# OmerKerner/noLZSS

Hardware: AMD Instinct MI355X
Metric: bases/sec factorized (1 GB sigma=4 DNA) + HBM GB/s fraction (higher is better)
Workload: dtype u32; 1 GPU; dna1g: one 2^30-base synthetic DNA sequence per GPU (sigma=4, 40% copied blocks, 1% substitutions), full factorization to (start,length,ref) records in HBM; bases_per_gpu=1073741824, parallelism=1 independent sequence shard(s), all-gather of counts

## Files before the change

nolzss_amd/csrc/chain.hip:

```cpp
#include "pipeline.hpp"
#include "pyramid.hpp"
#include "scan.hpp"

#include <cassert>

namespace nolzss {
namespace {

constexpr int kThreads = 256;
constexpr int kTile = 4096;
constexpr int kPerThread = kTile / kThreads;
constexpr uint32_t kNone = 0xffffffffu;

constexpr uint32_t kLenMask = 0x7fffffffu;

__device__ __forceinline__ uint32_t next_pos(uint32_t p, uint32_t code, uint32_t n) {
    const uint32_t L = code & kLenMask;
    const uint64_t nx = (uint64_t)p + (L ? L : 1u);
    return nx > n ? n : (uint32_t)nx;
}

__global__ __launch_bounds__(kThreads) void chain_exit_kernel(const uint32_t *__restrict__ lstar, uint32_t n,
                                                              uint32_t start_pos,
                                                              uint32_t *__restrict__ exit0,
                                                              uint32_t *__restrict__ target_bits) {
    __shared__ uint32_t jump[kTile];
    const uint32_t base = blockIdx.x * (uint32_t)kTile;
    const uint32_t tile_end = (n - base < (uint32_t)kTile) ? n : base + kTile;
    const int tid = threadIdx.x;
    uint32_t ls[kPerThread];
#pragma unroll
    for (int j = 0; j < kPerThread; ++j) {
        const uint32_t p = base + j * kThreads + tid;
        ls[j] = lstar[p < n ? p : n - 1u];
    }
#pragma unroll
    for (int j = 0; j < kPerThread; ++j) {
        const uint32_t lp = j * kThreads + tid;
        const uint32_t p = base + lp;
        jump[lp] = (p < n) ? next_pos(p, ls[j], n) : n;
    }
    __syncthreads();
    for (int round = 0; round < 13; ++round) {
        int changed = 0;
#pragma unroll
        for (int j = 0; j < kPerThread; ++j) {
            const uint32_t lp = j * kThreads + tid;
            const uint32_t t = jump[lp];
            if (t < tile_end) {
                jump[lp] = jump[t - base];
                changed = 1;
            }
        }
        if (!__syncthreads_or(changed)) break;
    }
#pragma unroll
    for (int j = 0; j < kPerThread; ++j) {
        const uint32_t lp = j * kThreads + tid;
        const uint32_t p = base + lp;
        if (p < n) {
            const uint32_t e = jump[lp];
            exit0[p] = e;
            const bool last = (lp + 1 == (uint32_t)kTile) || (p + 1 >= n);
            if (e < n && (last || jump[lp + 1] != e)) atomicOr(&target_bits[e >> 5], 1u << (e & 31));
        }
    }
    if (blockIdx.x == 0 && tid == 0 && start_pos < n) atomicOr(&target_bits[start_pos >> 5], 1u << (start_pos & 31));
}

__global__ __launch_bounds__(kThreads) void popcount_kernel(const uint32_t *__restrict__ bits, uint32_t nwords,
                                                            uint32_t *__restrict__ counts) {
    const size_t stride = (size_t)gridDim.x * blockDim.x;
    for (size_t w = (size_t)blockIdx.x * blockDim.x + threadIdx.x; w < nwords; w += stride)
        counts[w] = (uint32_t)__popc(bits[w]);
}

__global__ __launch_bounds__(kThreads) void node_fill_kernel(const uint32_t *__restrict__ bits,
                                                             const uint32_t *__restrict__ prefix, uint32_t nwords,
                                                             uint32_t *__restrict__ node_pos) {
    const size_t stride = (size_t)gridDim.x * blockDim.x;
    for (size_t w = (size_t)blockIdx.x * blockDim.x + threadIdx.x; w < nwords; w += stride) {
        uint32_t b = bits[w];
        uint32_t id = prefix[w];
        while (b) {
            const int bit = __ffs((int)b) - 1;
            node_pos[id++] = (uint32_t)(w * 32 + bit);
            b &= b - 1;
        }
    }
}

__device__ __forceinline__ uint32_t node_id(const uint32_t *bits, const uint32_t *prefix, uint32_t p) {
    return prefix[p >> 5] + (uint32_t)__popc(bits[p >> 5] & ((1u << (p & 31)) - 1u));
}

__global__ __launch_bounds__(kThreads) void node_edges_kernel(const uint32_t *__restrict__ node_pos, uint32_t K,
                                                              const uint32_t *__restrict__ exit0, uint32_t n,
                                                              const uint32_t *__restrict__ bits,
                                                              const uint32_t *__restrict__ prefix,
                                                              uint32_t start_pos, uint32_t *__restrict__ nxt,
                                                              uint32_t *__restrict__ reach) {
    const size_t stride = (size_t)gridDim.x * blockDim.x;
    for (size_t k = (size_t)blockIdx.x * blockDim.x + threadIdx.x; k <= K; k += stride) {
        if (k == K) {
            nxt[k] = K;
            reach[k] = 0;
            continue;
        }
        const uint32_t p = node_pos[k];
        const uint32_t e = exit0[p];
        nxt[k] = (e >= n) ? K : node_id(bits, prefix, e);
        reach[k] = (p == start_pos) ? 1u : 0u;
    }
}

__global__ __launch_bounds__(kThreads) void wyllie_kernel(const uint32_t *__restrict__ nxt_in,
                                                          uint32_t *__restrict__ nxt_out, uint32_t K,
                                                          uint32_t *reach) {
    const size_t stride = (size_t)gridDim.x * blockDim.x;
    for (size_t k = (size_t)blockIdx.x * blockDim.x + threadIdx.x; k < K; k += stride) {
        const uint32_t w = nxt_in[k];
        if (w < K) {
            if (reach[k]) reach[w] = 1u;
            nxt_out[k] = nxt_in[w];
        } else {
            nxt_out[k] = K;
        }
    }
}

__global__ __launch_bounds__(kThreads) void tile_entries_kernel(const uint32_t *__restrict__ node_pos,
                                                                const uint32_t *__restrict__ reach, uint32_t K,
                                                                uint32_t *__restrict__ entry) {
    const size_t stride = (size_t)gridDim.x * blockDim.x;
    for (size_t k = (size_t)blockIdx.x * blockDim.x + threadIdx.x; k < K; k += stride)
        if (reach[k]) {
            const uint32_t p = node_pos[k];
            entry[p / kTile] = p;
        }
}

__global__ __launch_bounds__(64) void chain_mark_kernel(const uint32_t *__restrict__ lstar, uint32_t n,
                                                        const uint32_t *__restrict__ entry,
                                                        unsigned long long *__restrict__ chain_bits,
                                                        uint32_t *__restrict__ tile_count) {
    __shared__ uint16_t jmp[kTile];
    __shared__ unsigned long long bits[kTile / 64];
    const uint32_t base = blockIdx.x * (uint32_t)kTile;
    const uint32_t tile_end = (n - base < (uint32_t)kTile) ? n : base + kTile;
    const int lane = threadIdx.x;
    const uint32_t e = entry[blockIdx.x];
    const size_t word0 = (size_t)blockIdx.x * (kTile / 64);
    if (e == kNone) {
        chain_bits[word0 + lane] = 0ull;
        if (lane == 0) tile_count[blockIdx.x] = 0;
        return;
    }
    constexpr int kBatch = 16;
    for (int j0 = 0; j0 < kTile / 64; j0 += kBatch) {
        uint32_t ls[kBatch];
#pragma unroll
        for (int j = 0; j < kBatch; ++j) {
            const uint32_t p = base + (uint32_t)(j0 + j) * 64u + lane;
            ls[j] = lstar[p < n ? p : n - 1u];
        }
#pragma unroll
        for (int j = 0; j < kBatch; ++j) {
            const uint32_t lp = (uint32_t)(j0 + j) * 64u + lane;
            const uint32_t p = base + lp;
            uint32_t nl = kTile;
            if (p < n) {
                const uint32_t nx = next_pos(p, ls[j], n);
                if (nx < tile_end) nl = nx - base;
            }
            jmp[lp] = (uint16_t)nl;
        }
    }
    bits[lane] = 0ull;
    __syncthreads();
    if (lane == 0) {
        uint32_t p = e - base, cnt = 0;
        while (p < (uint32_t)kTile) {
            bits[p >> 6] |= 1ull << (p & 63);
            ++cnt;
            p = jmp[p];
        }
        tile_count[blockIdx.x] = cnt;
    }
    __syncthreads();
    chain_bits[word0 + lane] = bits[lane];
}

__global__ __launch_bounds__(64) void emit_positions_kernel(const unsigned long long *__restrict__ chain_bits,
                                                            const uint32_t *__restrict__ tile_off,
                                                            uint32_t *__restrict__ fpos) {
    const int lane = threadIdx.x;
    const size_t word = (size_t)blockIdx.x * (kTile / 64) + lane;
    unsigned long long b = chain_bits[word];
    const uint32_t c = (uint32_t)__popcll(b);
    uint32_t off = wave_scan_inclusive(c, OpAdd<uint32_t>()) - c + tile_off[blockIdx.x];
    const uint32_t p0 = blockIdx.x * (uint32_t)kTile + lane * 64u;
    while (b) {
        const int bit = __ffsll((long long)b) - 1;
        fpos[off++] = p0 + (uint32_t)bit;
        b &= b - 1;
    }
}

template <bool kRC>
__global__ __launch_bounds__(kThreads) void length_hist_kernel(const unsigned long long *__restrict__ chain_bits,
                                                               uint32_t nwords, const uint32_t *__restrict__ lstar,
                                                               uint32_t *__restrict__ hist,
                                                               uint64_t *__restrict__ tail,
                                                               uint32_t *__restrict__ tail_count, uint32_t tail_cap) {
    constexpr uint32_t T = kLengthHistBins;
    constexpr uint32_t kBins = kRC ? 2 * T : T;
    __shared__ uint32_t h[kBins];
    for (uint32_t b = threadIdx.x; b < kBins; b += kThreads) h[b] = 0;
    __syncthreads();
    const uint32_t stride = gridDim.x * kThreads;
    for (uint32_t w = blockIdx.x * kThreads + threadIdx.x; w < nwords; w += stride) {
        unsigned long long b = chain_bits[w];
        while (b) {
            const int bit = __ffsll((long long)b) - 1;
            b &= b - 1;
            const uint32_t code = lstar[(size_t)w * 64 + (uint32_t)bit];
            const uint32_t strand = kRC ? (code >> 31) : 0u;
            uint32_t L = code & kLenMask;
            L = L ? L : 1u;
            if (L < T) {
                atomicAdd(&h[strand * T + L], 1u);
            } else {
                const uint32_t slot = atomicAdd(tail_count, 1u);
                assert(slot < tail_cap);
                if (slot < tail_cap) tail[slot] = (uint64_t)L | ((uint64_t)strand << 32);
            }
        }
    }
    __syncthreads();
    for (uint32_t b = threadIdx.x; b < kBins; b += kThreads)
        if (h[b]) atomicAdd(&hist[b], h[b]);
}

__global__ __launch_bounds__(kThreads) void gather_lengths_kernel(uint32_t *__restrict__ fpos, uint32_t z,
                                                                  const uint32_t *__restrict__ lstar) {
    const size_t stride = (size_t)gridDim.x * blockDim.x;
    for (size_t k = (size_t)blockIdx.x * blockDim.x + threadIdx.x; k < z; k += stride) {
        const uint32_t L = lstar[fpos[k]] & kLenMask;
        fpos[k] = L ? L : 1u;
    }
}

constexpr uint32_t kEmitScan = 4;

struct FactorRec {
    uint64_t start, length, ref;
};

template <bool kRC, bool kRebase>
__global__ __launch_bounds__(kThreads) void factor_kernel(const uint32_t *__restrict__ fpos, uint32_t z,
                                                          const uint32_t *__restrict__ lstar,
                                                          const uint32_t *__restrict__ isa,
                                                          const uint32_t *__restrict__ sa,
                                                          const uint32_t *__restrict__ lcp, Pyramid Psa,
                                                          Pyramid Plcp, Pyramid Pmax, uint32_t rcN,
                                                          FactorRec *__restrict__ out, TermTable terms, uint32_t n) {
    const size_t stride = (size_t)gridDim.x * blockDim.x;
    for (size_t k = (size_t)blockIdx.x * blockDim.x + threadIdx.x; k < z; k += stride) {
        const uint32_t i = fpos[k];
        const uint32_t nxt = k + 1 < z ? fpos[k + 1] : n;
        uint32_t code = nxt - i;
        if (kRC || code == 1u) code = lstar[i];
        const uint32_t L = code & kLenMask;
        const bool is_rc = kRC && (code >> 31);
        FactorRec f;
        f.start = i;
        if (L == 0) {
            f.length = 1;
            f.ref = i;
        } else {
            const uint32_t r = isa[i] - 1u;
            uint32_t lo = r, hi = r + 1, steps = 0;
            while (lcp[lo] >= L) {
                --lo;
                if (++steps == kEmitScan) {
                    lo = (uint32_t)pyr_nearest_left<false>(Plcp, lo, L);
                    break;
                }
            }
            steps = 0;
            while (lcp[hi] >= L) {
                ++hi;
                if (++steps == kEmitScan) {
                    hi = pyr_nearest_right<false>(Plcp, hi, L);
                    break;
                }
            }
            hi -= 1;
            f.length = L;
            if (!is_rc) {
                uint32_t mn;
                if (hi - lo < 2 * kEmitScan) {
                    mn = kNone;
                    for (uint32_t q = lo; q <= hi; ++q) {
                        const uint32_t v = sa[q];
                        mn = v < mn ? v : mn;
                    }
                } else {
                    mn = pyr_range<false>(Psa, lo, hi);
                }
                f.ref = mn;
            } else {
                uint32_t mx;
                if (hi - lo < 2 * kEmitScan) {
                    mx = 0;
                    for (uint32_t q = lo; q <= hi; ++q) {
                        const uint32_t v = sa[q];
                        mx = v > mx ? v : mx;
                    }
                } else {
                    mx = pyr_range<true>(Pmax, lo, hi);
                }
                const uint64_t end = 2ull * rcN - mx;
                f.ref = (1ull << 63) | (end - L + 1);
            }
        }
        if (kRebase) {
            const uint32_t t = term_lower_bound(terms, i);
            const uint64_t base = t ? (uint64_t)terms.pos[t - 1] + 1 : 0;
            f.start -= base;
            f.ref -= base;
        }
        out[k] = f;
    }
}

inline unsigned grid_for(size_t items, unsigned cap = 256u * 16u) {
    size_t g = div_up(items, (size_t)kThreads);
    if (g < 1) g = 1;
    return (unsigned)(g > cap ? cap : g);
}

}

uint32_t resolve_chain(Context &ctx, uint32_t n, uint32_t start_pos, const uint32_t *lstar, const uint32_t *sa,
                       const uint32_t *isa, const uint32_t *lcp, const Pyramid &Psa, const Pyramid &Plcp,
                       void **d_factors_out, uint32_t rcN, const Pyramid *Pmax, uint32_t **d_fpos_out,
                       const TermTable *rebase, const ChainLengthsOut *lengths) {
    hipStream_t s = ctx.stream;
    Arena &arena = ctx.arena;
    if (d_factors_out) *d_factors_out = nullptr;
    if (d_fpos_out) *d_fpos_out = nullptr;
    if (start_pos >= n) return 0;

    const uint32_t num_tiles = (uint32_t)div_up(n, kTile);
    const uint32_t tbits_words = (uint32_t)div_up((size_t)n + 1, 32);

    uint32_t *fpos = nullptr;
    const size_t mark = arena.mark();
    uint32_t *exit0 = arena.alloc<uint32_t>(n);
    uint32_t *tbits = arena.alloc<uint32_t>(tbits_words);
    uint32_t *tprefix = arena.alloc<uint32_t>(tbits_words);
    uint32_t *d_total = arena.alloc<uint32_t>(2);
    HIP_CHECK(hipMemsetAsync(tbits, 0, sizeof(uint32_t) * tbits_words, s));
    {
        ProfScope ps(ctx.profiler(), "chain_exit", s);
        chain_exit_kernel<<<num_tiles, kThreads, 0, s>>>(lstar, n, start_pos, exit0, tbits);
        KERNEL_CHECK();
    }
    {
        ProfScope ps(ctx.profiler(), "chain_nodes", s);
        popcount_kernel<<<grid_for(tbits_words), kThreads, 0, s>>>(tbits, tbits_words, tprefix);
        KERNEL_CHECK();
        scan_exclusive_add_u32(tprefix, tprefix, tbits_words, d_total, arena, s);
    }
    uint32_t K = 0;
    ctx.read_back(d_total, &K, 1);

    uint32_t *node_pos = arena.alloc<uint32_t>(K + 1);
    uint32_t *nxt[2] = {arena.alloc<uint32_t>(K + 1), arena.alloc<uint32_t>(K + 1)};
    uint32_t *reach = arena.alloc<uint32_t>(K + 1);
    uint32_t *entry = arena.alloc<uint32_t>(num_tiles);
    {
        ProfScope ps(ctx.profiler(), "chain_nodes", s);
        node_fill_kernel<<<grid_for(tbits_words), kThreads, 0, s>>>(tbits, tprefix, tbits_words, node_pos);
        KERNEL_CHECK();
        node_edges_kernel<<<grid_for((size_t)K + 1), kThreads, 0, s>>>(node_pos, K, exit0, n, tbits, tprefix,
                                                                       start_pos, nxt[0], reach);
        KERNEL_CHECK();
    }
    {
        ProfScope ps(ctx.profiler(), "chain_wyllie", s);
        int rounds = 1;
        while ((1ull << rounds) < (uint64_t)K + 1) ++rounds;
        int cur = 0;
        for (int r = 0; r < rounds; ++r) {
            wyllie_kernel<<<grid_for(K), kThreads, 0, s>>>(nxt[cur], nxt[cur ^ 1], K, reach);
            KERNEL_CHECK();
            cur ^= 1;
        }
        HIP_CHECK(hipMemsetAsync(entry, 0xff, sizeof(uint32_t) * num_tiles, s));
        tile_entries_kernel<<<grid_for(K), kThreads, 0, s>>>(node_pos, reach, K, entry);
        KERNEL_CHECK();
    }
    unsigned long long *cbits = arena.alloc<unsigned long long>((size_t)num_tiles * (kTile / 64));
    uint32_t *tile_count = arena.alloc<uint32_t>(num_tiles);
    {
        ProfScope ps(ctx.profiler(), "chain_mark", s);
        chain_mark_kernel<<<num_tiles, 64, 0, s>>>(lstar, n, entry, cbits, tile_count);
        KERNEL_CHECK();
        scan_exclusive_add_u32(tile_count, tile_count, num_tiles, d_total + 1, arena, s);
    }
    uint32_t z = 0;
    ctx.read_back(d_total + 1, &z, 1);
    if (lengths) {
        if (d_factors_out || d_fpos_out) throw HipError("resolve_chain: factor lengths come without records");
        if (lengths->hist && z) {
            ProfScope ps(ctx.profiler(), "length_hist", s);
            const uint32_t nwords = num_tiles * (uint32_t)(kTile / 64);
            const unsigned g = grid_for(nwords, 1024);
            if (rcN)
                length_hist_kernel<true><<<g, kThreads, 0, s>>>(cbits, nwords, lstar, lengths->hist, lengths->tail,
                                                                lengths->tail_count, lengths->tail_cap);
            else
                length_hist_kernel<false><<<g, kThreads, 0, s>>>(cbits, nwords, lstar, lengths->hist, lengths->tail,
                                                                 lengths->tail_count, lengths->tail_cap);
            KERNEL_CHECK();
        }
        if (!lengths->order || z == 0) {
            arena.rewind(mark);
            return z;
        }
        fpos = arena.alloc<uint32_t>(z);
        ProfScope ps(ctx.profiler(), "length_emit", s);
        emit_positions_kernel<<<num_tiles, 64, 0, s>>>(cbits, tile_count, fpos);
        KERNEL_CHECK();
        gather_lengths_kernel<<<grid_for(z), kThreads, 0, s>>>(fpos, z, lstar);
        KERNEL_CHECK();
        *lengths->order = fpos;
        return z;
    }
    if ((!d_factors_out && !d_fpos_out) || z == 0) {
        arena.rewind(mark);
        return z;
    }
    fpos = arena.alloc<uint32_t>(z);
    if (!d_factors_out) {
        ProfScope ps(ctx.profiler(), "factor_emit", s);
        emit_positions_kernel<<<num_tiles, 64, 0, s>>>(cbits, tile_count, fpos);
        KERNEL_CHECK();
        *d_fpos_out = fpos;
        return z;
    }
    FactorRec *recs_tmp = arena.alloc<FactorRec>(z);
    {
        ProfScope ps(ctx.profiler(), "factor_emit", s);
        emit_positions_kernel<<<num_tiles, 64, 0, s>>>(cbits, tile_count, fpos);
        KERNEL_CHECK();
        if (rcN) {
            if (rebase) throw HipError("resolve_chain: record-relative output exists in plain mode only");
            factor_kernel<true, false><<<grid_for(z), kThreads, 0, s>>>(fpos, z, lstar, isa, sa, lcp, Psa, Plcp, *Pmax,
                                                                        rcN, recs_tmp, TermTable{}, n);
        } else if (rebase) {
            factor_kernel<false, true><<<grid_for(z), kThreads, 0, s>>>(fpos, z, lstar, isa, sa, lcp, Psa, Plcp, Psa,
                                                                        0u, recs_tmp, *rebase, n);
        } else {
            factor_kernel<false, false><<<grid_for(z), kThreads, 0, s>>>(fpos, z, lstar, isa, sa, lcp, Psa, Plcp, Psa,
                                                                         0u, recs_tmp, TermTable{}, n);
        }
        KERNEL_CHECK();
    }
    *d_factors_out = recs_tmp;
    if (d_fpos_out) *d_fpos_out = fpos;
    return z;
}

}
```

Before: 13.31 billion bases/s.

## Emit factor references in rank order using shared-memory SA/LCP tiles

Adds a rank-ordered factor emission path. Factors are keyed by ISA rank and radix-sorted, then each block loads a tile of SA and LCP (with halos and per-block minima) into shared memory and resolves the previous-occurrence reference locally. It falls back to the global pyramids only when the search leaves the tile, and scatters the results back to factor order before assembling the records. The aim is to replace random global pyramid lookups with coalesced tile loads. The cost is an extra sort, a scatter pass and more arena memory.

```diff
diff --git a/nolzss_amd/csrc/chain.hip b/nolzss_amd/csrc/chain.hip
--- a/nolzss_amd/csrc/chain.hip
+++ b/nolzss_amd/csrc/chain.hip
@@ -1,8 +1,10 @@
 #include "pipeline.hpp"
 #include "pyramid.hpp"
+#include "radix_sort.hpp"
 #include "scan.hpp"
 
 #include <cassert>
+#include <cstdlib>
 
 namespace nolzss {
 namespace {
@@ -341,6 +343,300 @@
     return (unsigned)(g > cap ? cap : g);
 }
 
+constexpr int kRankTileBits = 13;
+constexpr int kRankTile = 1 << kRankTileBits;
+constexpr int kRankHalo = 256;
+constexpr int kRankSpan = kRankTile + 2 * kRankHalo;
+constexpr int kRankBlk = 16;
+constexpr int kRankBlocks = kRankSpan / kRankBlk;
+constexpr int kRankThreads = 512;
+constexpr uint32_t kLiteralKey = 0xffffffffu;
+constexpr uint32_t kRankMinN = kRankTile / 2;
+static_assert(kRankSpan % (4 * kRankBlk) == 0 && kRankHalo % kRankBlk == 0, "aligned blocks, 16-byte rows");
+
+__device__ __forceinline__ uint32_t factor_length(const uint32_t *__restrict__ fpos, uint32_t z, uint32_t k, uint32_t n,
+                                                  const uint32_t *__restrict__ lstar, uint32_t &i) {
+    i = fpos[k];
+    const uint32_t nxt = k + 1 < z ? fpos[k + 1] : n;
+    uint32_t code = nxt - i;
+    if (code == 1u) code = lstar[i];
+    return code & kLenMask;
+}
+
+__global__ __launch_bounds__(kThreads) void rank_keys_kernel(const uint32_t *__restrict__ fpos, uint32_t z, uint32_t n,
+                                                             const uint32_t *__restrict__ lstar,
+                                                             const uint32_t *__restrict__ isa, uint32_t kbits,
+                                                             uint32_t *__restrict__ keys, uint32_t *__restrict__ vals) {
+    const uint32_t esc = (uint32_t)((1ull << (32 - kbits)) - 1ull);
+    const size_t stride = (size_t)gridDim.x * blockDim.x;
+    for (size_t k = (size_t)blockIdx.x * blockDim.x + threadIdx.x; k < z; k += stride) {
+        uint32_t i;
+        const uint32_t L = factor_length(fpos, z, (uint32_t)k, n, lstar, i);
+        keys[k] = L ? isa[i] - 1u : kLiteralKey;
+        vals[k] = (uint32_t)k | (uint32_t)((uint64_t)(L < esc ? L : esc) << kbits);
+    }
+}
+
+__global__ __launch_bounds__(kThreads) void rank_bounds_kernel(const uint32_t *__restrict__ keys, uint32_t z, int shift,
+                                                               uint32_t groups, uint32_t *__restrict__ start) {
+    const size_t stride = (size_t)gridDim.x * blockDim.x;
+    for (size_t j = (size_t)blockIdx.x * blockDim.x + threadIdx.x; j < z; j += stride) {
+        const uint32_t g = (keys[j] >> shift) & (groups - 1u);
+        const uint32_t first = j ? ((keys[j - 1] >> shift) & (groups - 1u)) + 1u : 0u;
+        for (uint32_t t = first; t <= g; ++t) start[t] = (uint32_t)j;
+        if (j + 1 == z)
+            for (uint32_t t = g + 1; t <= groups; ++t) start[t] = z;
+    }
+}
+
+__device__ __forceinline__ uint32_t rank_lookup(const uint32_t *s_sa, const uint32_t *s_lcp, const uint32_t *b_sa,
+                                                const uint32_t *b_lcp, int li, uint32_t L, uint32_t r, int64_t first,
+                                                const Pyramid &Psa, const Pyramid &Plcp, uint32_t *far_count) {
+    int q = li;
+    bool far_l = false;
+    {
+        int B = q / kRankBlk;
+        const int stop = B * kRankBlk;
+        while (q >= stop && s_lcp[q] >= L) --q;
+        if (q < stop) {
+            --B;
+            while (B >= 0 && b_lcp[B] >= L) --B;
+            far_l = B < 0;
+            if (!far_l) {
+                q = B * kRankBlk + kRankBlk - 1;
+                while (s_lcp[q] >= L) --q;
+            }
+        }
+    }
+    int p = li + 1;
+    bool far_r = false;
+    {
+        int B = p / kRankBlk;
+        const int stop = (B + 1) * kRankBlk;
+        while (p < stop && s_lcp[p] >= L) ++p;
+        if (p == stop) {
+            ++B;
+            while (B <= kRankBlocks && b_lcp[B] >= L) ++B;
+            far_r = B > kRankBlocks;
+            if (!far_r) {
+                p = B * kRankBlk;
+                while (s_lcp[p] >= L) ++p;
+            }
+        }
+    }
+    uint32_t mn = kNone;
+    if (!far_l && !far_r) {
+        int a = q, b = p - 1;
+        if (b - a >= 2 * kRankBlk) {
+            for (; a % kRankBlk; ++a) mn = s_sa[a] < mn ? s_sa[a] : mn;
+            for (; b % kRankBlk != kRankBlk - 1; --b) mn = s_sa[b] < mn ? s_sa[b] : mn;
+            for (int B = a / kRankBlk; B <= b / kRankBlk; ++B) mn = b_sa[B] < mn ? b_sa[B] : mn;
+        } else {
+            for (; a <= b; ++a) mn = s_sa[a] < mn ? s_sa[a] : mn;
+        }
+    } else {
+        const uint32_t lo = far_l ? (uint32_t)pyr_nearest_left<false>(Plcp, r, L) : (uint32_t)(first + q);
+        const uint32_t hi = (far_r ? pyr_nearest_right<false>(Plcp, r + 1u, L) : (uint32_t)(first + p)) - 1u;
+        mn = pyr_range<false>(Psa, lo, hi);
+        if (far_count) atomicAdd(far_count, 1u);
+    }
+    return mn;
+}
+
+__global__ __launch_bounds__(kRankThreads, 4) void rank_tile_kernel(
+    const uint32_t *__restrict__ keys, const uint32_t *__restrict__ vals, const uint32_t *__restrict__ start, int sub_bits,
+    uint32_t kbits, const uint32_t *__restrict__ fpos, uint32_t z, const uint32_t *__restrict__ sa,
+    const uint32_t *__restrict__ lcp, uint32_t n, Pyramid Psa, Pyramid Plcp, uint32_t *__restrict__ out_k,
+    uint32_t *__restrict__ out_ref, uint32_t *far_count) {
+    __shared__ __attribute__((aligned(16))) uint32_t s_sa[kRankSpan];
+    __shared__ __attribute__((aligned(16))) uint32_t s_lcp[kRankSpan + kRankBlk];
+    __shared__ uint32_t b_sa[kRankBlocks];
+    __shared__ uint32_t b_lcp[kRankBlocks + 1];
+    const uint32_t tile = blockIdx.x;
+    const uint32_t j0 = start[tile >> sub_bits], j1 = start[(tile >> sub_bits) + 1u];
+    if (j0 == j1) return;
+    const bool lead = (tile & ((1u << sub_bits) - 1u)) == 0;
+    const uint64_t base = (uint64_t)tile << kRankTileBits;
+    const int tid = threadIdx.x;
+    if (base >= n) {
+        if (lead)
+            for (uint32_t j = j0 + tid; j < j1; j += kRankThreads)
+                if (keys[j] == kLiteralKey) {
+                    out_k[j] = vals[j] & (uint32_t)((1ull << kbits) - 1ull);
+                    out_ref[j] = 0;
+                }
+        return;
+    }
+    const int64_t first = (int64_t)base - kRankHalo;
+    const uint32_t jf = j0 + tid;
+    const uint32_t rf = jf < j1 ? keys[jf] : 0u, vf = jf < j1 ? vals[jf] : 0u;
+    {
+        constexpr int kVecs = kRankSpan / 4;
+        constexpr int kRows = (kVecs + kRankThreads - 1) / kRankThreads;
+        uint4 a[kRows], c[kRows];
+#pragma unroll
+        for (int k = 0; k < kRows; ++k) {
+            const int v = k * kRankThreads + tid;
+            const int64_t g = first + 4 * (int64_t)v;
+            const bool in_sa = v < kVecs && g >= 0 && g < (int64_t)n;
+            const bool in_lcp = v < kVecs && g >= 0 && g <= (int64_t)n;
+            a[k] = in_sa ? *reinterpret_cast<const uint4 *>(sa + (in_sa ? g : 0)) : make_uint4(kNone, kNone, kNone, kNone);
+            c[k] = in_lcp ? *reinterpret_cast<const uint4 *>(lcp + (in_lcp ? g : 0)) : make_uint4(0u, 0u, 0u, 0u);
+        }
+        uint32_t tail = kNone;
+        if (tid == 0) {
+            const int64_t g = first + kRankSpan;
+            tail = (g >= 0 && g <= (int64_t)n) ? lcp[g] : 0u;
+        }
+#pragma unroll
+        for (int k = 0; k < kRows; ++k) {
+            const int v = k * kRankThreads + tid;
+            const int64_t g = first + 4 * (int64_t)v;
+            if (v < kVecs) {
+                uint4 x = a[k], y = c[k];
+                if (g + 1 >= (int64_t)n) x.y = kNone;
+                if (g + 2 >= (int64_t)n) x.z = kNone;
+                if (g + 3 >= (int64_t)n) x.w = kNone;
+                if (g + 1 > (int64_t)n) y.y = 0u;
+                if (g + 2 > (int64_t)n) y.z = 0u;
+                if (g + 3 > (int64_t)n) y.w = 0u;
+                reinterpret_cast<uint4 *>(s_sa)[v] = x;
+                reinterpret_cast<uint4 *>(s_lcp)[v] = y;
+            }
+        }
+        if (tid < kRankBlk) s_lcp[kRankSpan + tid] = tail;
+    }
+    __syncthreads();
+    for (int B = tid; B <= kRankBlocks; B += kRankThreads) {
+        const uint4 *c = reinterpret_cast<const uint4 *>(s_lcp + kRankBlk * B);
+        uint32_t ml = kNone, ms = kNone;
+#pragma unroll
+        for (int e = 0; e < kRankBlk / 4; ++e) {
+            const uint4 y = c[e];
+            ml = min(min(ml, y.x), min(min(y.y, y.z), y.w));
+        }
+        b_lcp[B] = ml;
+        if (B < kRankBlocks) {
+            const uint4 *p = reinterpret_cast<const uint4 *>(s_sa + kRankBlk * B);
+#pragma unroll
+            for (int e = 0; e < kRankBlk / 4; ++e) {
+                const uint4 x = p[e];
+                ms = min(min(ms, x.x), min(min(x.y, x.z), x.w));
+            }
+            b_sa[B] = ms;
+        }
+    }
+    __syncthreads();
+    const uint32_t kmask = (uint32_t)((1ull << kbits) - 1ull);
+    const uint32_t esc = (uint32_t)((1ull << (32 - kbits)) - 1ull);
+    for (uint32_t j = j0 + tid; j < j1; j += kRankThreads) {
+        const uint32_t r = j == jf ? rf : keys[j], v = j == jf ? vf : vals[j];
+        const uint32_t k = v & kmask;
+        if (r == kLiteralKey) {
+            if (lead) {
+                out_k[j] = k;
+                out_ref[j] = 0;
+            }
+            continue;
+        }
+        if ((r >> kRankTileBits) != tile) continue;
+        uint32_t L = (uint32_t)((uint64_t)v >> kbits);
+        if (L == esc) L = (k + 1 < z ? fpos[k + 1] : n) - fpos[k];
+        out_k[j] = k;
+        out_ref[j] = rank_lookup(s_sa, s_lcp, b_sa, b_lcp, (int)(r - (uint32_t)base) + kRankHalo, L, r, first, Psa, Plcp,
+                                 far_count);
+    }
+}
+
+template <bool kRebase>
+__global__ __launch_bounds__(kThreads) void assemble_kernel(const uint32_t *__restrict__ fpos, uint32_t z, uint32_t n,
+                                                            const uint32_t *__restrict__ lstar,
+                                                            const uint32_t *__restrict__ ref32,
+                                                            FactorRec *__restrict__ out, TermTable terms) {
+    const size_t stride = (size_t)gridDim.x * blockDim.x;
+    for (size_t k = (size_t)blockIdx.x * blockDim.x + threadIdx.x; k < z; k += stride) {
+        uint32_t i;
+        const uint32_t L = factor_length(fpos, z, (uint32_t)k, n, lstar, i);
+        FactorRec f;
+        f.start = i;
+        f.length = L ? L : 1u;
+        f.ref = L ? ref32[k] : i;
+        if (kRebase) {
+            const uint32_t t = term_lower_bound(terms, i);
+            const uint64_t base = t ? (uint64_t)terms.pos[t - 1] + 1 : 0;
+            f.start -= base;
+            f.ref -= base;
+        }
+        out[k] = f;
+    }
+}
+
+const char *emit_rank_order(Context &ctx, uint32_t n, uint32_t z, const uint32_t *fpos, const uint32_t *lstar,
+                            const uint32_t *isa, const uint32_t *sa, const uint32_t *lcp, const Pyramid &Psa,
+                            const Pyramid &Plcp, FactorRec *recs, const TermTable *rebase) {
+    static const bool by_factor = getenv("NOLZSS_EMIT_BY_FACTOR") != nullptr && atoi(getenv("NOLZSS_EMIT_BY_FACTOR")) != 0;
+    static const bool trace = getenv("NOLZSS_TRACE") != nullptr;
+    if (by_factor) return "NOLZSS_EMIT_BY_FACTOR";
+    static const uint32_t min_n = getenv("NOLZSS_EMIT_RANK_MIN") ? (uint32_t)atoll(getenv("NOLZSS_EMIT_RANK_MIN")) : kRankMinN;
+    if (n < min_n) return "text below half a tile of ranks";
+    if (z > 0x80000000u) return "more than 2^31 factors";
+    if ((reinterpret_cast<uintptr_t>(sa) | reinterpret_cast<uintptr_t>(lcp)) & 15u) return "sa or lcp not 16-byte aligned";
+    hipStream_t s = ctx.stream;
+    Arena &arena = ctx.arena;
+    int nb = 1;
+    while (nb < 32 && (1ull << nb) < (uint64_t)n) ++nb;
+    const int gbits = nb > kRankTileBits ? nb - kRankTileBits : 1;
+    const int sub_bits = gbits == 2 * kRadixBits + 1 ? 1 : 0;
+    const int npasses = (int)div_up((size_t)(gbits - sub_bits), kRadixBits);
+    const int shift = kRankTileBits + sub_bits;
+    const uint32_t groups = 1u << (kRadixBits * npasses);
+    const size_t need = 5 * ((size_t)z * 4 + 256) + ((size_t)groups + 1) * 4 + 2 * (div_up(z, kSortTile) * 1024 + 256) +
+                        (size_t(1) << 20);
+    if (arena.capacity() - arena.mark() < need) return "not enough arena memory";
+    uint32_t kbits = 1;
+    while ((1ull << kbits) < (uint64_t)z) ++kbits;
+
+    uint32_t *keys[2] = {arena.alloc<uint32_t>(z), arena.alloc<uint32_t>(z)};
+    uint32_t *vals[2] = {arena.alloc<uint32_t>(z), arena.alloc<uint32_t>(z)};
+    uint32_t *ref32 = arena.alloc<uint32_t>(z);
+    uint32_t *start = arena.alloc<uint32_t>((size_t)groups + 1);
+    uint32_t *far_count = nullptr;
+    if (trace) {
+        far_count = arena.alloc<uint32_t>(1);
+        HIP_CHECK(hipMemsetAsync(far_count, 0, sizeof(uint32_t), s));
+    }
+    rank_keys_kernel<<<grid_for(z), kThreads, 0, s>>>(fpos, z, n, lstar, isa, kbits, keys[0], vals[0]);
+    KERNEL_CHECK();
+    int shifts[4];
+    for (int p = 0; p < npasses; ++p) shifts[p] = shift + kRadixBits * p;
+    const int cur = radix_sort_pairs(keys, vals, z, shifts, npasses, arena, s, nullptr);
+    rank_bounds_kernel<<<grid_for(z), kThreads, 0, s>>>(keys[cur], z, shift, groups, start);
+    KERNEL_CHECK();
+    const uint32_t tiles = groups << sub_bits;
+    rank_tile_kernel<<<tiles, kRankThreads, 0, s>>>(keys[cur], vals[cur], start, sub_bits, kbits, fpos, z, sa, lcp, n, Psa,
+                                                    Plcp, keys[cur ^ 1], vals[cur ^ 1], far_count);
+    KERNEL_CHECK();
+    {
+        uint32_t *idx[2] = {keys[cur ^ 1], keys[cur]};
+        uint32_t *val[2] = {vals[cur ^ 1], vals[cur]};
+        bucketed_scatter(idx, val, z, ref32, z, arena, s, nullptr, false);
+    }
+    if (rebase)
+        assemble_kernel<true><<<grid_for(z), kThreads, 0, s>>>(fpos, z, n, lstar, ref32, recs, *rebase);
+    else
+        assemble_kernel<false><<<grid_for(z), kThreads, 0, s>>>(fpos, z, n, lstar, ref32, recs, TermTable{});
+    KERNEL_CHECK();
+    if (trace) {
+        uint32_t far = 0;
+        ctx.read_back(far_count, &far, 1);
+        fprintf(stderr,
+                "[nolzss] factor_emit: rank order, %u factors, %u tiles of %d ranks, %d sort pass(es) by groups of %d tile(s), "
+                "%u lookups finished from global memory\n",
+                z, (uint32_t)div_up(n, kRankTile), kRankTile, npasses, 1 << sub_bits, far);
+    }
+    return nullptr;
+}
+
 }
 
 uint32_t resolve_chain(Context &ctx, uint32_t n, uint32_t start_pos, const uint32_t *lstar, const uint32_t *sa,
@@ -461,10 +757,14 @@
             if (rebase) throw HipError("resolve_chain: record-relative output exists in plain mode only");
             factor_kernel<true, false><<<grid_for(z), kThreads, 0, s>>>(fpos, z, lstar, isa, sa, lcp, Psa, Plcp, *Pmax,
                                                                         rcN, recs_tmp, TermTable{}, n);
+        } else if (const char *why = emit_rank_order(ctx, n, z, fpos, lstar, isa, sa, lcp, Psa, Plcp, recs_tmp, rebase);
+                   why == nullptr) {
         } else if (rebase) {
+            if (getenv("NOLZSS_TRACE")) fprintf(stderr, "[nolzss] factor_emit: by factor (%s), %u factors\n", why, z);
             factor_kernel<false, true><<<grid_for(z), kThreads, 0, s>>>(fpos, z, lstar, isa, sa, lcp, Psa, Plcp, Psa,
                                                                         0u, recs_tmp, *rebase, n);
         } else {
+            if (getenv("NOLZSS_TRACE")) fprintf(stderr, "[nolzss] factor_emit: by factor (%s), %u factors\n", why, z);
             factor_kernel<false, false><<<grid_for(z), kThreads, 0, s>>>(fpos, z, lstar, isa, sa, lcp, Psa, Plcp, Psa,
                                                                          0u, recs_tmp, TermTable{}, n);
         }
```

Result: slower. 12.18 billion bases/s (-8.5%).
